# peterWon/D-LIOM

Measured on AMD Instinct MI355X. Metric: scans/sec (64-beam x 1024 pts -> 10 cm 3D submap), higher is better.
Workload: dtype f32 transforms + u16 voxels/u64 sums (rtcsm), f64 (ceres); 1 GPU; config2 W-dense: 64x1024 scan, all returns matched (adaptive voxel filters neutralised), RTCSM3D + CeresScanMatcher3D(hi+lo) + insertion(hi+lo); N_hi=65536, N_lo=65536, C=35937, linear_window=1, angular_window=5, rescored_candidates_last=2, box_kernel_variant=0, map_scans=20, grids_inserted_into=2, parallelism=replicas x1

## Files before the change

### d-liom_amd/csrc/rtcsm3d.hip

```cpp
#include <algorithm>
#include <cmath>
#include <cstdlib>
#include <cstring>
#include <type_traits>
#include <vector>

#include <dlfcn.h>
#include <rccl/rccl.h>

#include "device_common.h"
#include "host_math.h"
#include "probability_values.h"
#include "score_box.h"

namespace dliom {

constexpr int kBlock = 256;

template <int PPT, bool WIDE = false>
__global__ __launch_bounds__(kBlock) void rtcsm_score_kernel(
    GridView g, const float* __restrict__ px, const float* __restrict__ py,
    const float* __restrict__ pz, const float4* __restrict__ rot, int R, int r_first, int r_last,
    const float* __restrict__ trans, int T, int rots_per_block,
    unsigned long long* __restrict__ sums) {
  extern __shared__ unsigned block_sum[];
  float x[PPT], y[PPT], z[PPT];
#pragma unroll
  for (int k = 0; k < PPT; ++k) {
    const int i = (blockIdx.x * PPT + k) * kBlock + threadIdx.x;
    x[k] = px[i];
    y[k] = py[i];
    z[k] = pz[i];
  }
  const int r_begin = r_first + blockIdx.y * rots_per_block;
  const int r_end = min(r_begin + rots_per_block, r_last);
  const int lane = threadIdx.x & 63;
  const float inv = g.inv_resolution;
  typedef typename std::conditional<WIDE, unsigned long long, unsigned>::type idx_t;
  const idx_t sentinel = static_cast<idx_t>(1) << (3 * g.log2_leaves);
  const unsigned lb = static_cast<unsigned>(g.log2_leaves);
  for (int r = r_begin; r < r_end; ++r) {
    for (int j = threadIdx.x; j < T; j += kBlock) block_sum[j] = 0u;
    __syncthreads();
    const float4 qq = rot[r];
// ... 578 lines not shown
    }
  }
  std::vector<unsigned> bitmap(static_cast<size_t>(passes) * kBitmapWords, 0u);
  const unsigned thr_units = static_cast<unsigned>(s_units + B);
  for (int tp = 0; tp < passes; ++tp) {
    const Pass& ps = pass[static_cast<size_t>(tp)];
    for (int a = 0; a < 3; ++a) {
      unsigned* words = bitmap.data() + static_cast<size_t>(tp) * kBitmapWords + static_cast<size_t>(a) * (kBuckets / 32);
      for (int jj = 0; jj < ps.tc; ++jj) {
        const double tv = static_cast<double>(tau[(static_cast<size_t>(tp) * TC + jj) * 4 + a]);
        const double af = tv - std::floor(tv);
        const double L = -af - 1.5 * u, H = -af + (thr_units + 1.5) * u;
        const long long b0 = static_cast<long long>(std::floor(L * kBuckets)), b1 = static_cast<long long>(std::floor(H * kBuckets));
        for (long long b = b0; b <= b1; ++b) {
          const unsigned m = static_cast<unsigned>(((b % kBuckets) + kBuckets) % kBuckets);
          words[m >> 5] |= 1u << (m & 31u);
        }
      }
    }
  }
  {
    const double step = c.w.angular_step_size;
    const double a_lanes = (2.0 * c.w.angular_window_size + 1.0) * step;
    const double spread = a_lanes * 0.6 * cloud.max_norm / res;
    const double dim = spread + 2.0 * taumax + 8.0;
    if (dim > kMaxDim || dim * dim * (dim * 0.25) > cells) return (ctx->last_box_refusal = DLIOM_BOX_REFUSED_WINDOW, DLIOM_ERR_CAPACITY);
  }
  const int rot_groups_all = (r_last - r_first + 63) / 64;
  static const int forced_nw = env_int("DLIOM_BOX_NW", 0);
  const int nw = forced_nw >= 1 && forced_nw <= kWaves
                     ? std::min(forced_nw, rot_groups_all)
                     : std::min(rot_groups_all, kWaves);
  const int rot_blocks = (rot_groups_all + nw - 1) / nw;
  if (TC * sizeof(float4) + kBitmapWords * 4 + 16 + static_cast<size_t>(nw) * kListWords * 4 + static_cast<size_t>(cells) * 2 >
      160 * 1024)
    return (ctx->last_box_refusal = DLIOM_BOX_REFUSED_LDS, DLIOM_ERR_CAPACITY);
  struct GroupCache {
    int A = -1, r_first = -1, r_last = -1, nw = 0;
    float step = 0.f;
    std::vector<Group> groups;
  };
  static thread_local GroupCache gcache;
  const bool gcache_hit = gcache.A == c.w.angular_window_size && gcache.step == c.w.angular_step_size &&
                          gcache.r_first == r_first && gcache.r_last == r_last && gcache.nw == nw;
  std::vector<Group>& groups = gcache.groups;
  if (!gcache_hit) {
    gcache.A = -1;
    groups.assign(static_cast<size_t>(rot_blocks), Group());
  }
  for (size_t gi = 0; !gcache_hit && gi < groups.size(); ++gi) {
    Group& gr = groups[gi];
    const int r0 = r_first + static_cast<int>(gi) * nw * 64;
    const int cnt = std::max(0, std::min(nw * 64, r_last - r0));
    gr.c_lane = cnt / 2;
    gr.theta2 = 0.f;
    for (int a = 0; a < 3; ++a) gr.dc[a] = gr.hd[a] = 0.f;
    if (cnt <= 0) {
      gr.c_lane = 0;
      continue;
    }
    auto qd = [&](int r, double q[4]) {
      const QF& f = c.rot_raw[static_cast<size_t>(r)];
      const double nn = std::sqrt(double(f.w) * f.w + double(f.x) * f.x + double(f.y) * f.y + double(f.z) * f.z);
      q[0] = f.w / nn; q[1] = f.x / nn; q[2] = f.y / nn; q[3] = f.z / nn;
    };
    double qc[4];
    qd(r0 + gr.c_lane, qc);
// ... 2 lines not shown
      double q[4];
      qd(r0 + l, q);
      const double a0 = qc[0], a1 = -qc[1], a2 = -qc[2], a3 = -qc[3];
      double dq[4] = {a0 * q[0] - a1 * q[1] - a2 * q[2] - a3 * q[3], a0 * q[1] + a1 * q[0] + a2 * q[3] - a3 * q[2],
                      a0 * q[2] - a1 * q[3] + a2 * q[0] + a3 * q[1], a0 * q[3] + a1 * q[2] - a2 * q[1] + a3 * q[0]};
      if (dq[0] < 0) for (double& v : dq) v = -v;
      const double vn = std::sqrt(dq[1] * dq[1] + dq[2] * dq[2] + dq[3] * dq[3]);
      const double ang = 2.0 * std::atan2(vn, dq[0]);
      const double k = vn > 1e-300 ? ang / vn : 2.0;
      const double dv[3] = {k * dq[1], k * dq[2], k * dq[3]};
      th = std::max(th, ang);
      for (int a = 0; a < 3; ++a) {
        lo3[a] = std::min(lo3[a], dv[a]);
        hi3[a] = std::max(hi3[a], dv[a]);
      }
    }
    if (th > 0.3) return (ctx->last_box_refusal = DLIOM_BOX_REFUSED_WINDOW, DLIOM_ERR_CAPACITY);
    for (int a = 0; a < 3; ++a) {
      gr.dc[a] = static_cast<float>(0.5 * (lo3[a] + hi3[a]));
      gr.hd[a] = static_cast<float>(0.5 * (hi3[a] - lo3[a]) * 1.0001 + 1e-7);
    }
    gr.theta2 = static_cast<float>(0.51 * th * th * 1.01 + 1e-9);
  }
  gcache.A = c.w.angular_window_size;
  gcache.step = c.w.angular_step_size;
  gcache.r_first = r_first;
  gcache.r_last = r_last;
  gcache.nw = nw;
  struct SpanGuard {
    dliom_ctx* c;
    int span;
    ~SpanGuard() { c->end_span(span); }
  } span_guard{ctx, ctx->begin_span(DLIOM_KERNEL_RTCSM_SCORE)};
  const size_t tau_bytes = align256(tau.size() * 4);
  const size_t pass_only_bytes = align256(pass.size() * sizeof(Pass));
  const size_t group_bytes = align256(groups.size() * sizeof(Group));
  const size_t bitmap_bytes = align256(bitmap.size() * 4);
  const size_t pass_bytes = pass_only_bytes + group_bytes + bitmap_bytes;
  DLIOM_TRY(ctx->box_tables.reserve(tau_bytes + pass_bytes));
  char* base = static_cast<char*>(ctx->box_tables.p);
  const Group* group_src = reinterpret_cast<const Group*>(base + tau_bytes + pass_only_bytes);
  if (tau_bytes + pass_bytes <= kPinBoxTables.bytes) {
    char* h = pinned_at<char>(ctx, kPinBoxTables);
    std::memcpy(h, tau.data(), tau.size() * 4);
    std::memcpy(h + tau_bytes, pass.data(), pass.size() * sizeof(Pass));
    std::memcpy(h + tau_bytes + pass_only_bytes, groups.data(), groups.size() * sizeof(Group));
    std::memcpy(h + tau_bytes + pass_only_bytes + group_bytes, bitmap.data(), bitmap.size() * 4);
    if (prep_add(prep, base, h, tau_bytes + pass_bytes, 0u))
      group_src = reinterpret_cast<const Group*>(h + tau_bytes + pass_only_bytes);
    else
      DLIOM_HIP_TRY(hipMemcpyAsync(base, h, tau_bytes + pass_bytes, hipMemcpyHostToDevice, ctx->stream));
  } else {
    DLIOM_HIP_TRY(hipMemcpyAsync(base, tau.data(), tau.size() * 4, hipMemcpyHostToDevice, ctx->stream));
    DLIOM_HIP_TRY(hipMemcpyAsync(base + tau_bytes, pass.data(), pass.size() * sizeof(Pass), hipMemcpyHostToDevice, ctx->stream));
    DLIOM_HIP_TRY(hipMemcpyAsync(base + tau_bytes + pass_only_bytes, groups.data(), groups.size() * sizeof(Group),
                                 hipMemcpyHostToDevice, ctx->stream));
    DLIOM_HIP_TRY(hipMemcpyAsync(base + tau_bytes + pass_only_bytes + group_bytes, bitmap.data(), bitmap.size() * 4,
                                 hipMemcpyHostToDevice, ctx->stream));
    DLIOM_HIP_TRY(hipStreamSynchronize(ctx->stream));
  }
  Params p;
  p.tau = reinterpret_cast<const float4*>(base);
  p.pass = reinterpret_cast<const Pass*>(base + tau_bytes);
  p.group = reinterpret_cast<const Group*>(base + tau_bytes + pass_only_bytes);
  p.bitmap = reinterpret_cast<const unsigned*>(base + tau_bytes + pass_only_bytes + group_bytes);
  p.trans = d.trans;
  p.rot = d.rot;
  p.sums = d_sums;
  p.error = d_error;
  p.R = R;
  p.r_first = r_first;
  p.r_last = r_last;
  p.T = T;
  p.passes = passes;
  p.n = n;
  p.chunk = std::min(kMaxChunk, std::max(4, chunk_pts & ~3));
  p.order = p.chunk == kCostChunk ? cloud.d_chunk_order : (p.chunk == kCostChunkBig ? cloud.d_chunk_order_big : nullptr);
  p.point_chunks = (n + p.chunk - 1) / p.chunk;
  const int rot_groups = (r_last - r_first + 63) / 64;
  p.rot_groups = rot_groups;
  p.rot_blocks = rot_blocks;
  p.nw = nw;
  p.thr = thr_units;
  p.cells = cells;
  static const int split_points = env_int("DLIOM_BOX_SPLIT", 1);
  p.split_points = split_points;
#ifdef DLIOM_EXPERIMENTS
  static const int box_debug = env_int("DLIOM_BOX_DEBUG", 0);
  p.debug = box_debug;
  if (box_debug & 512) p.order = nullptr;
#else
  p.debug = 0;
#endif
  const size_t lds = TC * sizeof(float4) + kBitmapWords * 4 + 16 + static_cast<size_t>(nw) * kListWords * 4 +
                     static_cast<size_t>(cells) * 2;
  if (lds > 160 * 1024) return (ctx->last_box_refusal = DLIOM_BOX_REFUSED_LDS, DLIOM_ERR_CAPACITY);
  typedef void (*BoxKernel)(GridView, Params, const float*, const float*, const float*);
  const BoxKernel kernel = variant == 0 ? rtcsm_score_box_kernel : (variant == 1 ? rtcsm_score_box_kernel_w3 : rtcsm_score_box_kernel_wide);
  const unsigned attr_bit = variant == 0 ? kFuncAttrScoreBox : (variant == 1 ? kFuncAttrScoreBoxW3 : kFuncAttrScoreBoxWide);
  if ((ctx->func_attr_set & attr_bit) == 0u) {
    DLIOM_HIP_TRY(hipFuncSetAttribute(reinterpret_cast<const void*>(kernel), hipFuncAttributeMaxDynamicSharedMemorySize, 160 * 1024));
    ctx->func_attr_set |= attr_bit;
  }
  ctx->last_box_variant = variant;
  static thread_local size_t resident_lds = 0;
  static thread_local int resident = 0, resident_nw = 0, resident_variant = -1;
  if (resident_lds != lds || resident_nw != nw || resident_variant != variant) {
    resident_nw = nw;
    resident_variant = variant;
    DLIOM_HIP_TRY(hipOccupancyMaxActiveBlocksPerMultiprocessor(&resident, reinterpret_cast<const void*>(kernel), 64 * nw, lds));
    resident_lds = lds;
  }
  const int want_blocks = std::max(1, resident) * ctx->num_cus;
  int slot_quads = std::max(1, want_blocks / std::max(1, rot_blocks * passes));
  slot_quads = std::min(slot_quads, p.point_chunks);
  p.slots = slot_quads;
  p.units = passes * rot_blocks;
  DLIOM_TRY(ctx->box_counters.reserve(static_cast<size_t>(passes) * rot_blocks * 4 + 256));
  if (!prep_add(prep, ctx->box_counters.p, nullptr, static_cast<size_t>(passes) * rot_blocks * 4, 0u))
    DLIOM_HIP_TRY(hipMemsetAsync(ctx->box_counters.p, 0, static_cast<size_t>(passes) * rot_blocks * 4, ctx->stream));
  p.counters = ctx->box_counters.as<unsigned>();
  p.ext_stride = static_cast<int>(cloud.n_padded);
  DLIOM_TRY(ctx->box_extents.reserve(static_cast<size_t>(rot_blocks) * 6 * static_cast<size_t>(cloud.n_padded) * 4));
  p.ext = ctx->box_extents.as<float>();
  {
    PrepArgs none;
    none.n = 0;
    const PrepArgs& jobs = prep != nullptr ? *prep : none;
    const unsigned prep_rows = jobs.n > 0 ? 1u : 0u;
    hipLaunchKernelGGL(rtcsm_box_extent_kernel, dim3(static_cast<unsigned>((n + 255) / 256), static_cast<unsigned>(rot_blocks) + prep_rows),
                       dim3(256), 0, ctx->stream, p, g.inv_resolution, cloud.d_xs, cloud.d_ys, cloud.d_zs, ctx->box_extents.as<float>(),
                       group_src, d.rot_src, jobs);
    if (prep != nullptr) prep->n = 0;
  }
  const unsigned blocks = static_cast<unsigned>(slot_quads) * passes * rot_blocks;
  hipLaunchKernelGGL(kernel, dim3(blocks), dim3(64 * nw), lds, ctx->stream, g, p, cloud.d_xs, cloud.d_ys, cloud.d_zs);
  DLIOM_HIP_TRY(hipGetLastError());
#ifdef DLIOM_TEST_HOOKS
  if (ctx->tuning[DLIOM_TUNE_RESERVED_TEST_HOOK] == 1) {
    ctx->tuning[DLIOM_TUNE_RESERVED_TEST_HOOK] = 0;
    DLIOM_HIP_TRY(hipMemsetAsync(static_cast<char*>(ctx->box_error.p) + 4, 1, 1, ctx->stream));
  }
#endif
  return DLIOM_OK;
}

constexpr int kScoreTargetBlocks = 8192;

static int launch_score_dense(dliom_ctx* ctx, const dliom_cloud& cloud, const GridView& g, const Candidates& c,
                              const DeviceCandidates& d, int r_first, int r_last, unsigned long long* d_sums,
                              int64_t* processed) {
  const int R = static_cast<int>(c.w.num_rotations), T = static_cast<int>(c.w.num_translations);
  const int n = static_cast<int>(cloud.n);
  const int Rs = r_last - r_first;
  const size_t trans_lds = static_cast<size_t>(T) * 16;
  if (trans_lds > 100 * 1024) return DLIOM_ERR_INVALID_ARGUMENT;
  int bs = kDenseMaxBlock;
  for (int cand = kDenseMaxBlock; cand >= 64; cand -= 64)
    if ((Rs + cand - 1) / cand * cand < (Rs + bs - 1) / bs * bs) bs = cand;
  if (static_cast<int64_t>((Rs + bs - 1) / bs) * ((n + 63) / 64) < 256) bs = 64;
  const int rot_groups = (Rs + bs - 1) / bs;
  int chunk = 4096;
  while (chunk > 8 && static_cast<int64_t>(rot_groups) * ((n + chunk - 1) / chunk) < kScoreTargetBlocks) chunk >>= 1;
  const int point_chunks = (n + chunk - 1) / chunk;
  *processed = static_cast<int64_t>(point_chunks) * chunk;
  DenseDomain dom;
  dom.lo = 0;
  dom.size = g.dense_stride;
// ... 753 lines not shown
```

### d-liom_amd/csrc/score_box.h

```cpp
#ifndef DLIOM_CSRC_SCORE_BOX_H_
#define DLIOM_CSRC_SCORE_BOX_H_

#include "device_common.h"

namespace dliom {
namespace box {

constexpr int kTC = 27;
#if !defined(DLIOM_EXPERIMENTS) || !defined(DLIOM_BOX_TC_WIDE)
#undef DLIOM_BOX_TC_WIDE
#define DLIOM_BOX_TC_WIDE 49
#endif
constexpr int kTCWide = DLIOM_BOX_TC_WIDE;
#if !defined(DLIOM_EXPERIMENTS) || !defined(DLIOM_BOX_MAX_WAVES)
#undef DLIOM_BOX_MAX_WAVES
#define DLIOM_BOX_MAX_WAVES 4
#endif
constexpr int kWaves = DLIOM_BOX_MAX_WAVES;
constexpr int kMaxDim = 120;
constexpr int kMaxChunk = 64;
constexpr int kBuckets = 8192;
constexpr int kBitmapWords = 3 * kBuckets / 32;
constexpr int kL1Cap = 320;
constexpr int kL2Cap = 128;
#ifndef DLIOM_BOX_HOT_P
#define DLIOM_BOX_HOT_P 4
#endif
constexpr int kHotP = DLIOM_BOX_HOT_P;
#if !defined(DLIOM_EXPERIMENTS) || !defined(DLIOM_BOX_EXP)
#undef DLIOM_BOX_EXP
#define DLIOM_BOX_EXP 0
#endif
#ifdef DLIOM_EXPERIMENTS
#define DLIOM_BOX_DBG(p, bit) (((p).debug & (bit)) != 0)
#define DLIOM_BOX_STAT(p, cond, k, v)                                                                \
  do {                                                                                                \
    if (((p).debug & 128) && (cond)) atomicAdd((p).error + 8 + (k), static_cast<unsigned>(v));        \
  } while (0)
#else
#define DLIOM_BOX_DBG(p, bit) false
#define DLIOM_BOX_STAT(p, cond, k, v) do { } while (0)
#endif
#ifndef DLIOM_BOX_PIPE
#define DLIOM_BOX_PIPE 1
#endif
#ifndef DLIOM_BOX_LATE_ACC
#define DLIOM_BOX_LATE_ACC 1
#endif
constexpr int kPipe = DLIOM_BOX_PIPE;
constexpr bool kLateAcc = DLIOM_BOX_LATE_ACC != 0;
constexpr int kRecords = 8;
constexpr int kListTrash = kL1Cap + kL2Cap + 4 * kRecords;
constexpr int kListWords = kListTrash + 4;

struct Pass {
  int gi[3];
  float f[3];
  float uc[3];
  float reach[3];
  int tc;
  int j0;
  int pad[2];
};

struct Group {
  int c_lane;
  float dc[3];
  float hd[3];
  float theta2;
};

struct Params {
  const float4* tau;
  const Pass* pass;
  const unsigned* bitmap;
  const float* trans;
  const float4* rot;
  const Group* group;
  const float* ext;
  int ext_stride;
  unsigned long long* sums;
  const unsigned* order;
  unsigned* counters;
  unsigned* error;
  int R, r_first, r_last, T, passes;
  int n;
  int chunk;
  int point_chunks, rot_groups, rot_blocks, nw, slots;
  int units;
  unsigned thr;
  int cells;
  int split_points;
  int debug;
};

typedef __attribute__((address_space(3))) const unsigned short lds_cu16;

__device__ __forceinline__ unsigned min_lo16(unsigned running, float w) {
  unsigned r;
  asm("v_min_u32_sdwa %0, %1, %2 dst_sel:DWORD dst_unused:UNUSED_PAD src0_sel:DWORD src1_sel:WORD_0"
      : "=v"(r)
      : "v"(running), "v"(w));
  return r;
}
__device__ __forceinline__ unsigned mad_hi16(float w, unsigned m, unsigned a) {
  unsigned r;
  asm("v_mad_u32_u16 %0, %1, %2, %3 op_sel:[1,0,0,0]" : "=v"(r) : "v"(w), "v"(m), "v"(a));
  return r;
}
typedef float float2v __attribute__((ext_vector_type(2)));
__device__ __forceinline__ float2v pk_add_lo(float2v a, float2v t) {
  float2v r;
  asm("v_pk_add_f32 %0, %1, %2 op_sel_hi:[1,0]" : "=v"(r) : "v"(a), "v"(t));
  return r;
}
__device__ __forceinline__ float2v pk_add_hi(float2v a, float2v t) {
  float2v r;
  asm("v_pk_add_f32 %0, %1, %2 op_sel:[0,1] op_sel_hi:[1,1]" : "=v"(r) : "v"(a), "v"(t));
  return r;
}
__device__ __forceinline__ unsigned to_vgpr(unsigned s) {
  unsigned v;
  asm volatile("v_mov_b32 %0, %1" : "=v"(v) : "s"(s));
  return v;
}
__device__ __forceinline__ float to_vgpr_f(float s) {
  float v;
// ... 41 lines not shown
                                           const float* __restrict__ px, const float* __restrict__ py,
                                           const float* __restrict__ pz, const Lists& ls, int base1, int n2, int rot0,
                                           int lane) {
  DLIOM_BOX_STAT(p, lane == 0, 6, n2);
  for (int e0 = 0; e0 < n2; e0 += 64) {
    const int e = e0 + lane;
    if (e < n2) {
      const unsigned item = ls.l2[e];
      const unsigned ent = ls.l1[base1 + static_cast<int>(item & 0xFFu)];
      const int j = static_cast<int>(item >> 8);
      const int* rc = ls.rec + 4 * static_cast<int>((ent >> 12) & (kRecords - 1));
      const int r = rot0 + static_cast<int>(ent & 63u), pt = rc[3] + static_cast<int>((ent >> 6) & 63u);
      const float4 qq = p.rot[r];
      const Quat4 q{qq.x, qq.y, qq.z, qq.w};
      float rx, ry, rz;
      rotate_point(q, px[pt], py[pt], pz[pt], rx, ry, rz);
      const float4 t = lds_tau[j];
      const float ax = __builtin_fmaf(rx, g.inv_resolution, static_cast<float>(ps.gi[0] - rc[0]) + ps.f[0]) + t.x;
      const float ay = __builtin_fmaf(ry, g.inv_resolution, static_cast<float>(ps.gi[1] - rc[1]) + ps.f[1]) + t.y;
      const float az = __builtin_fmaf(rz, g.inv_resolution, static_cast<float>(ps.gi[2] - rc[2]) + ps.f[2]) + t.z;
      const int fx = static_cast<int>((__float_as_uint(ax) >> 16) - 0x4300u) + rc[0];
      const int fy = static_cast<int>((__float_as_uint(ay) >> 16) - 0x4300u) + rc[1];
      const int fz = static_cast<int>((__float_as_uint(az) >> 16) - 0x4300u) + rc[2];
      const float* tr = p.trans + 3 * (ps.j0 + j);
      const int ex = cell_of(rx + tr[0], g.resolution), ey = cell_of(ry + tr[1], g.resolution),
                ez = cell_of(rz + tr[2], g.resolution);
      if (ex != fx || ey != fy || ez != fz) {
        if (abs(ex - fx) > 1 || abs(ey - fy) > 1 || abs(ez - fz) > 1) {
          atomicOr(p.error, 1u);
          atomicOr(p.error + 1, 1u);
        }
        const long long delta = static_cast<long long>(mirror_value(g, ex, ey, ez)) -
                                static_cast<long long>(mirror_value(g, fx, fy, fz));
        if (delta != 0)
          atomicAdd(&p.sums[static_cast<size_t>(ps.j0 + j) * p.R + r], static_cast<unsigned long long>(delta));
      }
    }
  }
}

__device__ __forceinline__ void resolve_l1(const GridView& g, const Params& p, const Pass& ps, const float4* lds_tau,
                                           const float* __restrict__ px, const float* __restrict__ py,
                                           const float* __restrict__ pz, const Lists& ls, int base1, int count, int rot0,
                                           int lane) {
  const bool have = lane < count;
  DLIOM_BOX_STAT(p, lane == 0, 4, 1);
  DLIOM_BOX_STAT(p, lane == 0, 5, count);
  float wx = 200.5f, wy = 200.5f, wz = 200.5f;
  if (have) {
    const unsigned ent = ls.l1[base1 + lane];
    const int* rc = ls.rec + 4 * static_cast<int>((ent >> 12) & (kRecords - 1));
    const int r = rot0 + static_cast<int>(ent & 63u), pt = rc[3] + static_cast<int>((ent >> 6) & 63u);
    const float4 qq = p.rot[r];
    const Quat4 q{qq.x, qq.y, qq.z, qq.w};
    float rx, ry, rz;
    rotate_point(q, px[pt], py[pt], pz[pt], rx, ry, rz);
    wx = __builtin_fmaf(rx, g.inv_resolution, static_cast<float>(ps.gi[0] - rc[0]) + ps.f[0]);
    wy = __builtin_fmaf(ry, g.inv_resolution, static_cast<float>(ps.gi[1] - rc[1]) + ps.f[1]);
    wz = __builtin_fmaf(rz, g.inv_resolution, static_cast<float>(ps.gi[2] - rc[2]) + ps.f[2]);
  }
  int n2 = 0;
  for (int j = 0; j < ps.tc; ++j) {
    const float4 t = lds_tau[j];
    unsigned m = min_lo16(0xFFFFFFFFu, wx + t.x);
    m = min_lo16(m, wy + t.y);
    m = min_lo16(m, wz + t.z);
    const bool mine = have && m <= p.thr;
    const unsigned long long mask = __builtin_amdgcn_ballot_w64(mine);
// ... 178 lines not shown
        acc[j - kPipe] += s;
        asm volatile("" : "+v"(acc[j - kPipe]));
      }
      if (kLateAcc) __builtin_amdgcn_sched_barrier(0);
      unsigned v[P];
#if DLIOM_BOX_EXP == 1
#pragma unroll
      for (int k = 0; k < P; ++k) v[k] = a[k] & 0x7fffu;
#else
#pragma unroll
      for (int k = 0; k < P; ++k) v[k] = *reinterpret_cast<lds_cu16*>(a[k]);
#endif
#pragma unroll
      for (int d = kPipe - 1; d > 0; --d)
#pragma unroll
        for (int k = 0; k < P; ++k) pv[d][k] = pv[d - 1][k];
#pragma unroll
      for (int k = 0; k < P; ++k) pv[0][k] = v[k];
      t = tn;
      __builtin_amdgcn_sched_barrier(0);
    }
#pragma unroll
    for (int d = kPipe - 1; d >= 0; --d) {
      unsigned s = pv[d][0];
#pragma unroll
      for (int k = 1; k < P; ++k) s += pv[d][k];
      acc[TC - 1 - d] += s;
      asm volatile("" : "+v"(acc[TC - 1 - d]));
    }
  }
  return i;
}

constexpr int kFlushPoints = 131072;
template <int TC>
__device__ __forceinline__ void flush_acc(const Params& p, const Pass& ps, unsigned (&acc)[TC], int r, bool lane_active) {
#pragma unroll
  for (int j = 0; j < TC; ++j) {
    if (lane_active && j < ps.tc && acc[j] != 0u)
      atomicAdd(&p.sums[static_cast<size_t>(ps.j0 + j) * p.R + r], static_cast<unsigned long long>(acc[j]));
    acc[j] = 0u;
  }
}

__device__ __forceinline__ bool box_geometry(const GridView& g, const Params& p, const Pass& ps, const float (&l3)[3],
                                             const float (&h3)[3], int n, int lane, Geometry& geo) {
  const bool have = lane < n;
  bool fits = true;
#pragma unroll
  for (int a = 0; a < 3; ++a) {
    const float l = fmaxf(wave_min_f(have ? l3[a] : 3.0e38f) - ps.reach[a], -1.0e6f);
    const float h = fminf(wave_max_f(have ? h3[a] : -3.0e38f) + ps.reach[a], 1.0e6f);
    geo.lo[a] = __builtin_amdgcn_readfirstlane(static_cast<int>(floorf(l)));
    geo.dim[a] = __builtin_amdgcn_readfirstlane(static_cast<int>(floorf(h))) - geo.lo[a] + 1;
  }
  {
    const int m_lo = (geo.lo[0] + g.dense_off[0]) & ~3;
    const int m_hi = geo.lo[0] + g.dense_off[0] + geo.dim[0];
    geo.lo[0] = m_lo - g.dense_off[0];
    geo.dim[0] = ((m_hi - m_lo) + 3) & ~3;
  }
  geo.sx = static_cast<unsigned>(geo.dim[0]);
  if (((geo.sx >> 2) & 1u) == 0u) geo.sx += 4u;
  const unsigned sy = static_cast<unsigned>(geo.dim[1]) | 1u;
  geo.sxy = geo.sx * sy;
#pragma unroll
  for (int a = 0; a < 3; ++a) {
    fits = fits && geo.dim[a] <= kMaxDim && abs(ps.gi[a] - geo.lo[a]) < 1000;
    geo.kb[a] = static_cast<float>(ps.gi[a] - geo.lo[a]) + ps.f[a];
  }
  fits = fits && static_cast<long long>(geo.sxy) * geo.dim[2] <= p.cells && geo.sxy <= 32767u;
  return fits;
}
// ... 29 lines not shown
    rabs[4] = fabsf(1.f - 2.f * (x * x + z * z));
    rabs[5] = fabsf(2.f * (y * z - w * x));
    rabs[6] = fabsf(2.f * (x * z - w * y));
    rabs[7] = fabsf(2.f * (y * z + w * x));
    rabs[8] = fabsf(1.f - 2.f * (x * x + y * y));
  }
  const float x = px[i], y = py[i], z = pz[i];
  const float sx_ = grp.dc[1] * z - grp.dc[2] * y, sy_ = grp.dc[2] * x - grp.dc[0] * z, sz_ = grp.dc[0] * y - grp.dc[1] * x;
  float cx, cy, cz;
  rotate_point(qc, x + sx_, y + sy_, z + sz_, cx, cy, cz);
  const float fx = fabsf(x), fy = fabsf(y), fz = fabsf(z);
  const float hx = grp.hd[1] * fz + grp.hd[2] * fy, hy = grp.hd[2] * fx + grp.hd[0] * fz, hz = grp.hd[0] * fy + grp.hd[1] * fx;
  const float m2 = grp.theta2 * (fx + fy + fz) + 1.0e-5f * (fx + fy + fz);
  const float c3[3] = {cx, cy, cz};
  float* out = ext + static_cast<size_t>(rb) * 6 * p.ext_stride + i;
#pragma unroll
  for (int a = 0; a < 3; ++a) {
    const float he = rabs[3 * a] * hx + rabs[3 * a + 1] * hy + rabs[3 * a + 2] * hz + m2;
    out[static_cast<size_t>(2 * a) * p.ext_stride] = (c3[a] - he) * inv;
    out[static_cast<size_t>(2 * a + 1) * p.ext_stride] = (c3[a] + he) * inv;
  }
}

template <int TC>
__device__ __forceinline__ void score_box_body(const GridView& g, const Params& p, const float* __restrict__ px,
                                               const float* __restrict__ py, const float* __restrict__ pz) {
  extern __shared__ float4 lds_dyn4[];
  float4* lds_tau = lds_dyn4;
  unsigned* lds_bitmap = reinterpret_cast<unsigned*>(lds_dyn4 + TC);
  const int wave = __builtin_amdgcn_readfirstlane(static_cast<int>(threadIdx.x >> 6)), lane = threadIdx.x & 63, nthreads = blockDim.x;
  typedef __attribute__((address_space(3))) char lds_char;
  const unsigned lds0 = static_cast<unsigned>(reinterpret_cast<size_t>((lds_char*)lds_dyn4));
  const unsigned tick_off = static_cast<unsigned>(TC * sizeof(float4)) + kBitmapWords * 4u;
  const unsigned lists_off = tick_off + 16u;
  const unsigned box_off = lists_off + static_cast<unsigned>(p.nw) * kListWords * 4u;
  const unsigned box_base = lds0 + box_off;
  unsigned short* box = reinterpret_cast<unsigned short*>(reinterpret_cast<char*>(lds_dyn4) + box_off);
  unsigned* tick = reinterpret_cast<unsigned*>(reinterpret_cast<char*>(lds_dyn4) + tick_off);
  Lists ls;
  ls.l1 = reinterpret_cast<unsigned*>(reinterpret_cast<char*>(lds_dyn4) + lists_off) + wave * kListWords;
  ls.l2 = ls.l1 + kL1Cap;
  ls.rec = reinterpret_cast<int*>(ls.l2 + kL2Cap);
  ls.n1 = 0;
  ls.seq = 0;
  unsigned acc[TC];
#pragma unroll
  for (int j = 0; j < TC; ++j) acc[j] = 0u;
  const int S = g.dense_stride, B = g.dense_bricks;
#ifdef DLIOM_EXPERIMENTS
  unsigned long long stamp_begin = 0ull;
  unsigned stamp_tickets = 0u;
  if (DLIOM_BOX_DBG(p, 256)) stamp_begin = wall_clock64();
#endif
  const int home = static_cast<int>(blockIdx.x % static_cast<unsigned>(p.units));
  const int slot = static_cast<int>(blockIdx.x / static_cast<unsigned>(p.units));
  int parity = 0;
  int loaded_pass = -1;
  const int hops = DLIOM_BOX_DBG(p, 64) ? 1 : p.units;
  for (int hop = 0; hop < hops; ++hop) {
    int unit = home + hop;
    if (unit >= p.units) unit -= p.units;
    unsigned* counter = p.counters + unit;
    int ticket, chunk_id;
    if (hop == 0) {
      ticket = DLIOM_BOX_DBG(p, 8) ? p.point_chunks : slot;
      chunk_id = (p.order != nullptr && ticket < p.point_chunks) ? static_cast<int>(p.order[ticket]) : ticket;
    } else {
      if (threadIdx.x == 0) {
        const int t = p.slots + static_cast<int>(atomicAdd(counter, 1u));
        tick[parity] = static_cast<unsigned>(t);
        tick[2 + parity] = (p.order != nullptr && t < p.point_chunks) ? p.order[t] : static_cast<unsigned>(t);
      }
      __syncthreads();
      ticket = static_cast<int>(tick[parity]);
      chunk_id = static_cast<int>(tick[2 + parity]);
      parity ^= 1;
    }
    if (ticket >= p.point_chunks) continue;
    const int rb = unit % p.rot_blocks;
    const int tp = unit / p.rot_blocks;
    if (tp != loaded_pass) {
      __syncthreads();
      if (threadIdx.x < TC) lds_tau[threadIdx.x] = p.tau[tp * TC + threadIdx.x];
      for (int w = threadIdx.x; w < kBitmapWords; w += nthreads) lds_bitmap[w] = p.bitmap[tp * kBitmapWords + w];
      __syncthreads();
      loaded_pass = tp;
    }
    const int rot_b0 = p.r_first + rb * p.nw * 64;
    const int groups_here = (p.r_last - rot_b0 + 63) >> 6;
    const int split = (p.split_points != 0 && p.nw == 4) ? (groups_here == 1 ? 4 : (groups_here == 2 ? 2 : 1)) : 1;
    const int rot_group = split == 4 ? 0 : (split == 2 ? (wave & 1) : wave);
    const int slice = split == 4 ? wave : (split == 2 ? (wave >> 1) : 0);
    const int rot0 = rot_b0 + rot_group * 64;
    const bool wave_active = rot0 < p.r_last && slice < split;
    const Pass ps = p.pass[tp];
    const bool lane_active = rot0 + lane < p.r_last;
    const float4 qq = p.rot[lane_active ? rot0 + lane : (wave_active ? rot0 : rot_b0)];
    const Quat4 q{qq.x, qq.y, qq.z, qq.w};
    const float* ext_rb = p.ext + static_cast<size_t>(rb) * 6 * p.ext_stride;
    int n_guess = p.chunk;
    int since_flush = 0;
    while (ticket < p.point_chunks) {
      unsigned next_raw = 0u, next_chunk = 0u;
      bool drawn = false;
#ifdef DLIOM_EXPERIMENTS
      ++stamp_tickets;
#endif
      {
        const int c = __builtin_amdgcn_readfirstlane(chunk_id);
        const int c_begin = c * p.chunk, c_end = min(c_begin + p.chunk, p.n);
        int lo = c_begin;
// ... 41 lines not shown
          DLIOM_BOX_STAT(p, threadIdx.x == 0, 0, 1);
          DLIOM_BOX_STAT(p, threadIdx.x == 0, 1, (geo.dim[0] >> 2) * geo.dim[1] * geo.dim[2]);
          DLIOM_BOX_STAT(p, threadIdx.x == 0, 2, n);
          __syncthreads();
          if (!DLIOM_BOX_DBG(p, 2)) {
            const unsigned quads = static_cast<unsigned>(geo.dim[0]) >> 2, dim1 = static_cast<unsigned>(geo.dim[1]);
            const unsigned total = __umul24(__umul24(quads, dim1), static_cast<unsigned>(geo.dim[2]));
            const float inv_q = 1.0f / static_cast<float>(quads), inv_dy = 1.0f / static_cast<float>(dim1);
            const int bx0 = geo.lo[0] + g.dense_off[0], by0 = geo.lo[1] + g.dense_off[1], bz0 = geo.lo[2] + g.dense_off[2];
            const unsigned uB = static_cast<unsigned>(B), uBB = __umul24(uB, uB), uS = static_cast<unsigned>(S);
            const char* dense_bytes = reinterpret_cast<const char*>(g.dense);
#pragma unroll 4
            for (unsigned e = threadIdx.x; e < total; e += static_cast<unsigned>(nthreads)) {
              const unsigned row = static_cast<unsigned>((static_cast<float>(e) + 0.5f) * inv_q);
              const unsigned xq = e - __umul24(row, quads);
              const unsigned z = static_cast<unsigned>((static_cast<float>(row) + 0.5f) * inv_dy);
              const unsigned y = row - __umul24(z, dim1);
              const int mx = bx0 + static_cast<int>(4u * xq), my = by0 + static_cast<int>(y), mz = bz0 + static_cast<int>(z);
              unsigned long long val = 0x0001000100010001ull;
              if (static_cast<unsigned>(mx) < 4u * uB && static_cast<unsigned>(my) < uS && static_cast<unsigned>(mz) < uS) {
                const unsigned umx = static_cast<unsigned>(mx), umy = static_cast<unsigned>(my), umz = static_cast<unsigned>(mz);
                const unsigned off = ((__umul24(umz >> 2, uBB) + __umul24(umy >> 2, uB) + (umx >> 2)) << 7) |
                                     (((umz & 3u) << 5) | ((umy & 3u) << 3));
                val = *reinterpret_cast<const unsigned long long*>(dense_bytes + off);
              }
              *reinterpret_cast<unsigned long long*>(box + (__umul24(z, geo.sxy) + __umul24(y, geo.sx) + 4u * xq)) = val;
            }
          }
          const unsigned rec_id = static_cast<unsigned>(ls.seq & (kRecords - 1));
          if (lane < 4) ls.rec[4 * rec_id + lane] = lane < 3 ? geo.lo[lane] : lo;
          ++ls.seq;
          __syncthreads();
          if (drawn && threadIdx.x == 0) {
            const int t = p.slots + static_cast<int>(next_raw);
            next_chunk = (p.order != nullptr && t < p.point_chunks) ? p.order[t] : static_cast<unsigned>(t);
          }
          if (wave_active && !DLIOM_BOX_DBG(p, 4)) {
            const int part = split > 1 ? ((((n + split - 1) >> (split == 4 ? 2 : 1)) + 3) & ~3) : n;
            const int s_lo = lo + min(n, slice * part), s_n = min(n, (slice + 1) * part) - min(n, slice * part);
            int i = s_lo;
            const int e8 = kHotP == 8 ? s_lo + (s_n & ~7) : s_lo, e4 = s_lo + (s_n & ~3), e1 = s_lo + s_n;
            for (;;) {
              if (kHotP == 8 && i < e8)
                i = main_loop<kHotP, TC>(g, p, geo, q, px, py, pz, i, e8, lo, lds_tau, lds_bitmap, box_base, ls, rec_id, lane_active, lane, acc);
              if (i >= e8 && i < e4)
                i = main_loop<4, TC>(g, p, geo, q, px, py, pz, i, e4, lo, lds_tau, lds_bitmap, box_base, ls, rec_id, lane_active, lane, acc);
              if (i >= e4 && i < e1)
                i = main_loop<1, TC>(g, p, geo, q, px, py, pz, i, e1, lo, lds_tau, lds_bitmap, box_base, ls, rec_id, lane_active, lane, acc);
              if (i >= e1) break;
              drain_l1(g, p, ps, lds_tau, px, py, pz, ls, false, rot0, lane);
            }
            if (!DLIOM_BOX_DBG(p, 1) && (ls.n1 >= 64 || (ls.seq & (kRecords - 1)) == 0))
              drain_l1(g, p, ps, lds_tau, px, py, pz, ls, (ls.seq & (kRecords - 1)) == 0, rot0, lane);
          }
          lo += n;
        }
      }
      if (threadIdx.x == 0) {
        if (!drawn) {
          const int t = p.slots + static_cast<int>(atomicAdd(counter, 1u));
          next_raw = static_cast<unsigned>(t - p.slots);
          next_chunk = (p.order != nullptr && t < p.point_chunks) ? p.order[t] : static_cast<unsigned>(t);
        }
        tick[parity] = static_cast<unsigned>(p.slots) + next_raw;
        tick[2 + parity] = next_chunk;
      }
      __syncthreads();
      ticket = static_cast<int>(tick[parity]);
      chunk_id = static_cast<int>(tick[2 + parity]);
      parity ^= 1;
    }
    if (wave_active && !DLIOM_BOX_DBG(p, 1)) drain_l1(g, p, ps, lds_tau, px, py, pz, ls, true, rot0, lane);
    ls.n1 = 0;
    if (DLIOM_BOX_DBG(p, 16)) {
#pragma unroll
      for (int j = 0; j < TC; ++j) {
        if (lane_active && j < ps.tc)
          atomicAdd(&p.sums[static_cast<size_t>(ps.j0 + j) * p.R + rot0 + lane], static_cast<unsigned long long>(acc[j]));
        acc[j] = 0u;
      }
    } else if (!DLIOM_BOX_DBG(p, 32)) {
      flush_acc(p, ps, acc, rot0 + lane, lane_active);
    }
  }
#ifdef DLIOM_EXPERIMENTS
  if (DLIOM_BOX_DBG(p, 256) && threadIdx.x == 0 && blockIdx.x < 4096u) {
    unsigned long long* st = reinterpret_cast<unsigned long long*>(p.error + 64) + 4 * blockIdx.x;
    unsigned xcc;
    asm volatile("s_getreg_b32 %0, hwreg(HW_REG_XCC_ID)" : "=s"(xcc));
    st[0] = stamp_begin;
    st[1] = wall_clock64();
    st[2] = stamp_tickets;
    st[3] = xcc;
  }
#endif
}


__global__ __launch_bounds__(64 * kWaves) __attribute__((amdgpu_waves_per_eu(4, 8))) void rtcsm_score_box_kernel(
    GridView g, Params p, const float* __restrict__ px, const float* __restrict__ py, const float* __restrict__ pz) {
  score_box_body<kTC>(g, p, px, py, pz);
}
__global__ __launch_bounds__(64 * kWaves) __attribute__((amdgpu_waves_per_eu(3, 8))) void rtcsm_score_box_kernel_w3(
    GridView g, Params p, const float* __restrict__ px, const float* __restrict__ py, const float* __restrict__ pz) {
  score_box_body<kTC>(g, p, px, py, pz);
}
__global__ __launch_bounds__(64 * kWaves) __attribute__((amdgpu_waves_per_eu(3, 8))) void rtcsm_score_box_kernel_wide(
    GridView g, Params p, const float* __restrict__ px, const float* __restrict__ py, const float* __restrict__ pz) {
  score_box_body<kTCWide>(g, p, px, py, pz);
}

}
}

#endif
```

Measured before the change: 965.6 scans/s.

## Weight-proportional block homes and dynamic work stealing across score-box units

Replaces the uniform slot-per-unit launch layout with a host-computed table that gives each (pass, rotation-block) unit a number of resident blocks proportional to its estimated work. A small home table is uploaded with the other box tables. When a block finishes its unit, it now picks the unit with the most remaining chunks instead of hopping round-robin. The change also switches sum atomics to 32-bit when the point count guarantees no overflow. The intent is to cut load imbalance and tail idle time, at the cost of extra host-side allotment, a per-unit scan of global counters by wave 0, and more atomic contention on busy units.

```diff
diff --git a/d-liom_amd/csrc/rtcsm3d.hip b/d-liom_amd/csrc/rtcsm3d.hip
--- a/d-liom_amd/csrc/rtcsm3d.hip
+++ b/d-liom_amd/csrc/rtcsm3d.hip
@@ -10,6 +10,7 @@
 
 #include "device_common.h"
 #include "host_math.h"
+#include "score_units.h"
 #include "probability_values.h"
 #include "score_box.h"
 
@@ -654,7 +655,7 @@
                      ? std::min(forced_nw, rot_groups_all)
                      : std::min(rot_groups_all, kWaves);
   const int rot_blocks = (rot_groups_all + nw - 1) / nw;
-  if (TC * sizeof(float4) + kBitmapWords * 4 + 16 + static_cast<size_t>(nw) * kListWords * 4 + static_cast<size_t>(cells) * 2 >
+  if (TC * sizeof(float4) + kBitmapWords * 4 + kTickBytes + static_cast<size_t>(nw) * kListWords * 4 + static_cast<size_t>(cells) * 2 >
       160 * 1024)
     return (ctx->last_box_refusal = DLIOM_BOX_REFUSED_LDS, DLIOM_ERR_CAPACITY);
   struct GroupCache {
@@ -723,38 +724,7 @@
     int span;
     ~SpanGuard() { c->end_span(span); }
   } span_guard{ctx, ctx->begin_span(DLIOM_KERNEL_RTCSM_SCORE)};
-  const size_t tau_bytes = align256(tau.size() * 4);
-  const size_t pass_only_bytes = align256(pass.size() * sizeof(Pass));
-  const size_t group_bytes = align256(groups.size() * sizeof(Group));
-  const size_t bitmap_bytes = align256(bitmap.size() * 4);
-  const size_t pass_bytes = pass_only_bytes + group_bytes + bitmap_bytes;
-  DLIOM_TRY(ctx->box_tables.reserve(tau_bytes + pass_bytes));
-  char* base = static_cast<char*>(ctx->box_tables.p);
-  const Group* group_src = reinterpret_cast<const Group*>(base + tau_bytes + pass_only_bytes);
-  if (tau_bytes + pass_bytes <= kPinBoxTables.bytes) {
-    char* h = pinned_at<char>(ctx, kPinBoxTables);
-    std::memcpy(h, tau.data(), tau.size() * 4);
-    std::memcpy(h + tau_bytes, pass.data(), pass.size() * sizeof(Pass));
-    std::memcpy(h + tau_bytes + pass_only_bytes, groups.data(), groups.size() * sizeof(Group));
-    std::memcpy(h + tau_bytes + pass_only_bytes + group_bytes, bitmap.data(), bitmap.size() * 4);
-    if (prep_add(prep, base, h, tau_bytes + pass_bytes, 0u))
-      group_src = reinterpret_cast<const Group*>(h + tau_bytes + pass_only_bytes);
-    else
-      DLIOM_HIP_TRY(hipMemcpyAsync(base, h, tau_bytes + pass_bytes, hipMemcpyHostToDevice, ctx->stream));
-  } else {
-    DLIOM_HIP_TRY(hipMemcpyAsync(base, tau.data(), tau.size() * 4, hipMemcpyHostToDevice, ctx->stream));
-    DLIOM_HIP_TRY(hipMemcpyAsync(base + tau_bytes, pass.data(), pass.size() * sizeof(Pass), hipMemcpyHostToDevice, ctx->stream));
-    DLIOM_HIP_TRY(hipMemcpyAsync(base + tau_bytes + pass_only_bytes, groups.data(), groups.size() * sizeof(Group),
-                                 hipMemcpyHostToDevice, ctx->stream));
-    DLIOM_HIP_TRY(hipMemcpyAsync(base + tau_bytes + pass_only_bytes + group_bytes, bitmap.data(), bitmap.size() * 4,
-                                 hipMemcpyHostToDevice, ctx->stream));
-    DLIOM_HIP_TRY(hipStreamSynchronize(ctx->stream));
-  }
   Params p;
-  p.tau = reinterpret_cast<const float4*>(base);
-  p.pass = reinterpret_cast<const Pass*>(base + tau_bytes);
-  p.group = reinterpret_cast<const Group*>(base + tau_bytes + pass_only_bytes);
-  p.bitmap = reinterpret_cast<const unsigned*>(base + tau_bytes + pass_only_bytes + group_bytes);
   p.trans = d.trans;
   p.rot = d.rot;
   p.sums = d_sums;
@@ -783,7 +753,7 @@
 #else
   p.debug = 0;
 #endif
-  const size_t lds = TC * sizeof(float4) + kBitmapWords * 4 + 16 + static_cast<size_t>(nw) * kListWords * 4 +
+  const size_t lds = TC * sizeof(float4) + kBitmapWords * 4 + kTickBytes + static_cast<size_t>(nw) * kListWords * 4 +
                      static_cast<size_t>(cells) * 2;
   if (lds > 160 * 1024) return (ctx->last_box_refusal = DLIOM_BOX_REFUSED_LDS, DLIOM_ERR_CAPACITY);
   typedef void (*BoxKernel)(GridView, Params, const float*, const float*, const float*);
@@ -805,8 +775,59 @@
   const int want_blocks = std::max(1, resident) * ctx->num_cus;
   int slot_quads = std::max(1, want_blocks / std::max(1, rot_blocks * passes));
   slot_quads = std::min(slot_quads, p.point_chunks);
-  p.slots = slot_quads;
+  p.add32 = n <= kFlushPoints ? 1 : 0;
   p.units = passes * rot_blocks;
+  std::vector<double> unit_weights(static_cast<size_t>(p.units));
+  for (int u = 0; u < p.units; ++u) {
+    const int rot_b0 = r_first + (u % rot_blocks) * nw * 64;
+    unit_weights[static_cast<size_t>(u)] = unit_weight((r_last - rot_b0 + 63) >> 6, nw, p.split_points);
+  }
+  std::vector<int> slots_per_unit;
+  std::vector<UnitHome> homes;
+  const unsigned blocks = static_cast<unsigned>(allot_homes(unit_weights, slot_quads * p.units, p.point_chunks, &slots_per_unit, &homes));
+  std::vector<unsigned> unit_slots(static_cast<size_t>(unit_slots_words(p.units)), 0u);
+  for (int u = 0; u < p.units; ++u) unit_slots[static_cast<size_t>(u)] = static_cast<unsigned>(slots_per_unit[static_cast<size_t>(u)]);
+  const size_t tau_bytes = align256(tau.size() * 4);
+  const size_t pass_only_bytes = align256(pass.size() * sizeof(Pass));
+  const size_t group_bytes = align256(groups.size() * sizeof(Group));
+  const size_t bitmap_bytes = align256(bitmap.size() * 4);
+  static_assert((kBitmapWords * 4) % 256 == 0 && sizeof(UnitHome) == 8, "unit_slots() finds the table behind the bitmaps");
+  const size_t unit_slot_bytes = static_cast<size_t>(unit_slots_words(p.units)) * 4;
+  const size_t unit_bytes = align256(unit_slot_bytes + homes.size() * sizeof(UnitHome));
+  const size_t pass_bytes = pass_only_bytes + group_bytes + bitmap_bytes + unit_bytes;
+  DLIOM_TRY(ctx->box_tables.reserve(tau_bytes + pass_bytes));
+  char* base = static_cast<char*>(ctx->box_tables.p);
+  const Group* group_src = reinterpret_cast<const Group*>(base + tau_bytes + pass_only_bytes);
+  if (tau_bytes + pass_bytes <= kPinBoxTables.bytes) {
+    char* h = pinned_at<char>(ctx, kPinBoxTables);
+    std::memcpy(h, tau.data(), tau.size() * 4);
+    std::memcpy(h + tau_bytes, pass.data(), pass.size() * sizeof(Pass));
+    std::memcpy(h + tau_bytes + pass_only_bytes, groups.data(), groups.size() * sizeof(Group));
+    std::memcpy(h + tau_bytes + pass_only_bytes + group_bytes, bitmap.data(), bitmap.size() * 4);
+    std::memcpy(h + tau_bytes + pass_only_bytes + group_bytes + bitmap_bytes, unit_slots.data(), unit_slots.size() * 4);
+    std::memcpy(h + tau_bytes + pass_only_bytes + group_bytes + bitmap_bytes + unit_slot_bytes, homes.data(),
+                homes.size() * sizeof(UnitHome));
+    if (prep_add(prep, base, h, tau_bytes + pass_bytes, 0u))
+      group_src = reinterpret_cast<const Group*>(h + tau_bytes + pass_only_bytes);
+    else
+      DLIOM_HIP_TRY(hipMemcpyAsync(base, h, tau_bytes + pass_bytes, hipMemcpyHostToDevice, ctx->stream));
+  } else {
+    DLIOM_HIP_TRY(hipMemcpyAsync(base, tau.data(), tau.size() * 4, hipMemcpyHostToDevice, ctx->stream));
+    DLIOM_HIP_TRY(hipMemcpyAsync(base + tau_bytes, pass.data(), pass.size() * sizeof(Pass), hipMemcpyHostToDevice, ctx->stream));
+    DLIOM_HIP_TRY(hipMemcpyAsync(base + tau_bytes + pass_only_bytes, groups.data(), groups.size() * sizeof(Group),
+                                 hipMemcpyHostToDevice, ctx->stream));
+    DLIOM_HIP_TRY(hipMemcpyAsync(base + tau_bytes + pass_only_bytes + group_bytes, bitmap.data(), bitmap.size() * 4,
+                                 hipMemcpyHostToDevice, ctx->stream));
+    DLIOM_HIP_TRY(hipMemcpyAsync(base + tau_bytes + pass_only_bytes + group_bytes + bitmap_bytes, unit_slots.data(),
+                                 unit_slots.size() * 4, hipMemcpyHostToDevice, ctx->stream));
+    DLIOM_HIP_TRY(hipMemcpyAsync(base + tau_bytes + pass_only_bytes + group_bytes + bitmap_bytes + unit_slot_bytes, homes.data(),
+                                 homes.size() * sizeof(UnitHome), hipMemcpyHostToDevice, ctx->stream));
+    DLIOM_HIP_TRY(hipStreamSynchronize(ctx->stream));
+  }
+  p.tau = reinterpret_cast<const float4*>(base);
+  p.pass = reinterpret_cast<const Pass*>(base + tau_bytes);
+  p.group = reinterpret_cast<const Group*>(base + tau_bytes + pass_only_bytes);
+  p.bitmap = reinterpret_cast<const unsigned*>(base + tau_bytes + pass_only_bytes + group_bytes);
   DLIOM_TRY(ctx->box_counters.reserve(static_cast<size_t>(passes) * rot_blocks * 4 + 256));
   if (!prep_add(prep, ctx->box_counters.p, nullptr, static_cast<size_t>(passes) * rot_blocks * 4, 0u))
     DLIOM_HIP_TRY(hipMemsetAsync(ctx->box_counters.p, 0, static_cast<size_t>(passes) * rot_blocks * 4, ctx->stream));
@@ -824,7 +845,6 @@
                        group_src, d.rot_src, jobs);
     if (prep != nullptr) prep->n = 0;
   }
-  const unsigned blocks = static_cast<unsigned>(slot_quads) * passes * rot_blocks;
   hipLaunchKernelGGL(kernel, dim3(blocks), dim3(64 * nw), lds, ctx->stream, g, p, cloud.d_xs, cloud.d_ys, cloud.d_zs);
   DLIOM_HIP_TRY(hipGetLastError());
 #ifdef DLIOM_TEST_HOOKS
diff --git a/d-liom_amd/csrc/score_box.h b/d-liom_amd/csrc/score_box.h
--- a/d-liom_amd/csrc/score_box.h
+++ b/d-liom_amd/csrc/score_box.h
@@ -52,6 +52,7 @@
 constexpr int kRecords = 8;
 constexpr int kListTrash = kL1Cap + kL2Cap + 4 * kRecords;
 constexpr int kListWords = kListTrash + 4;
+constexpr int kTickBytes = 32;
 
 struct Pass {
   int gi[3];
@@ -86,13 +87,24 @@
   int R, r_first, r_last, T, passes;
   int n;
   int chunk;
-  int point_chunks, rot_groups, rot_blocks, nw, slots;
+  int point_chunks, rot_groups, rot_blocks, nw;
+  int add32;
   int units;
   unsigned thr;
   int cells;
   int split_points;
   int debug;
 };
+
+__host__ __device__ __forceinline__ int unit_slots_words(int units) { return (units + 3) & ~3; }
+__device__ __forceinline__ const unsigned* unit_slots(const Params& p) { return p.bitmap + p.passes * kBitmapWords; }
+__device__ __forceinline__ const uint2* unit_homes(const Params& p) {
+  return reinterpret_cast<const uint2*>(unit_slots(p) + unit_slots_words(p.units));
+}
+
+constexpr int kFlushPoints = 131072;
+static_assert(static_cast<unsigned long long>(kFlushPoints) * 0x7fffull <= 0xffffffffull,
+              "kFlushPoints values of at most 0x7fff (the mask of a grid value) fit an accumulator and a 32-bit sum");
 
 typedef __attribute__((address_space(3))) const unsigned short lds_cu16;
 
@@ -200,8 +212,13 @@
         }
         const long long delta = static_cast<long long>(mirror_value(g, ex, ey, ez)) -
                                 static_cast<long long>(mirror_value(g, fx, fy, fz));
-        if (delta != 0)
-          atomicAdd(&p.sums[static_cast<size_t>(ps.j0 + j) * p.R + r], static_cast<unsigned long long>(delta));
+        if (delta != 0) {
+          unsigned long long* sum = &p.sums[static_cast<size_t>(ps.j0 + j) * p.R + r];
+          if (p.add32 != 0)
+            atomicAdd(reinterpret_cast<unsigned*>(sum), static_cast<unsigned>(delta));
+          else
+            atomicAdd(sum, static_cast<unsigned long long>(delta));
+        }
       }
     }
   }
@@ -446,13 +463,18 @@
   return i;
 }
 
-constexpr int kFlushPoints = 131072;
 template <int TC>
 __device__ __forceinline__ void flush_acc(const Params& p, const Pass& ps, unsigned (&acc)[TC], int r, bool lane_active) {
+  const bool add32 = p.add32 != 0;
 #pragma unroll
   for (int j = 0; j < TC; ++j) {
-    if (lane_active && j < ps.tc && acc[j] != 0u)
-      atomicAdd(&p.sums[static_cast<size_t>(ps.j0 + j) * p.R + r], static_cast<unsigned long long>(acc[j]));
+    if (lane_active && j < ps.tc && acc[j] != 0u) {
+      unsigned long long* sum = &p.sums[static_cast<size_t>(ps.j0 + j) * p.R + r];
+      if (add32)
+        atomicAdd(reinterpret_cast<unsigned*>(sum), acc[j]);
+      else
+        atomicAdd(sum, static_cast<unsigned long long>(acc[j]));
+    }
     acc[j] = 0u;
   }
 }
@@ -548,7 +570,7 @@
   typedef __attribute__((address_space(3))) char lds_char;
   const unsigned lds0 = static_cast<unsigned>(reinterpret_cast<size_t>((lds_char*)lds_dyn4));
   const unsigned tick_off = static_cast<unsigned>(TC * sizeof(float4)) + kBitmapWords * 4u;
-  const unsigned lists_off = tick_off + 16u;
+  const unsigned lists_off = tick_off + static_cast<unsigned>(kTickBytes);
   const unsigned box_off = lists_off + static_cast<unsigned>(p.nw) * kListWords * 4u;
   const unsigned box_base = lds0 + box_off;
   unsigned short* box = reinterpret_cast<unsigned short*>(reinterpret_cast<char*>(lds_dyn4) + box_off);
@@ -565,34 +587,21 @@
   const int S = g.dense_stride, B = g.dense_bricks;
 #ifdef DLIOM_EXPERIMENTS
   unsigned long long stamp_begin = 0ull;
-  unsigned stamp_tickets = 0u;
+  unsigned stamp_tickets = 0u, stamp_visits = 0u;
   if (DLIOM_BOX_DBG(p, 256)) stamp_begin = wall_clock64();
 #endif
-  const int home = static_cast<int>(blockIdx.x % static_cast<unsigned>(p.units));
-  const int slot = static_cast<int>(blockIdx.x / static_cast<unsigned>(p.units));
+  int unit, ticket, chunk_id;
+  {
+    const uint2 home = unit_homes(p)[blockIdx.x];
+    unit = static_cast<int>(home.x);
+    ticket = DLIOM_BOX_DBG(p, 8) ? p.point_chunks : static_cast<int>(home.y);
+    chunk_id = (p.order != nullptr && ticket < p.point_chunks) ? static_cast<int>(p.order[ticket]) : ticket;
+  }
   int parity = 0;
   int loaded_pass = -1;
-  const int hops = DLIOM_BOX_DBG(p, 64) ? 1 : p.units;
-  for (int hop = 0; hop < hops; ++hop) {
-    int unit = home + hop;
-    if (unit >= p.units) unit -= p.units;
+  for (;;) {
     unsigned* counter = p.counters + unit;
-    int ticket, chunk_id;
-    if (hop == 0) {
-      ticket = DLIOM_BOX_DBG(p, 8) ? p.point_chunks : slot;
-      chunk_id = (p.order != nullptr && ticket < p.point_chunks) ? static_cast<int>(p.order[ticket]) : ticket;
-    } else {
-      if (threadIdx.x == 0) {
-        const int t = p.slots + static_cast<int>(atomicAdd(counter, 1u));
-        tick[parity] = static_cast<unsigned>(t);
-        tick[2 + parity] = (p.order != nullptr && t < p.point_chunks) ? p.order[t] : static_cast<unsigned>(t);
-      }
-      __syncthreads();
-      ticket = static_cast<int>(tick[parity]);
-      chunk_id = static_cast<int>(tick[2 + parity]);
-      parity ^= 1;
-    }
-    if (ticket >= p.point_chunks) continue;
+    const int slots_u = static_cast<int>(unit_slots(p)[unit]);
     const int rb = unit % p.rot_blocks;
     const int tp = unit / p.rot_blocks;
     if (tp != loaded_pass) {
@@ -700,7 +709,7 @@
           ++ls.seq;
           __syncthreads();
           if (drawn && threadIdx.x == 0) {
-            const int t = p.slots + static_cast<int>(next_raw);
+            const int t = slots_u + static_cast<int>(next_raw);
             next_chunk = (p.order != nullptr && t < p.point_chunks) ? p.order[t] : static_cast<unsigned>(t);
           }
           if (wave_active && !DLIOM_BOX_DBG(p, 4)) {
@@ -726,18 +735,21 @@
       }
       if (threadIdx.x == 0) {
         if (!drawn) {
-          const int t = p.slots + static_cast<int>(atomicAdd(counter, 1u));
-          next_raw = static_cast<unsigned>(t - p.slots);
+          const int t = slots_u + static_cast<int>(atomicAdd(counter, 1u));
+          next_raw = static_cast<unsigned>(t - slots_u);
           next_chunk = (p.order != nullptr && t < p.point_chunks) ? p.order[t] : static_cast<unsigned>(t);
         }
-        tick[parity] = static_cast<unsigned>(p.slots) + next_raw;
+        tick[parity] = static_cast<unsigned>(slots_u) + next_raw;
         tick[2 + parity] = next_chunk;
       }
       __syncthreads();
-      ticket = static_cast<int>(tick[parity]);
+      ticket = __builtin_amdgcn_readfirstlane(static_cast<int>(tick[parity]));
       chunk_id = static_cast<int>(tick[2 + parity]);
       parity ^= 1;
     }
+#ifdef DLIOM_EXPERIMENTS
+    ++stamp_visits;
+#endif
     if (wave_active && !DLIOM_BOX_DBG(p, 1)) drain_l1(g, p, ps, lds_tau, px, py, pz, ls, true, rot0, lane);
     ls.n1 = 0;
     if (DLIOM_BOX_DBG(p, 16)) {
@@ -750,6 +762,38 @@
     } else if (!DLIOM_BOX_DBG(p, 32)) {
       flush_acc(p, ps, acc, rot0 + lane, lane_active);
     }
+    if (DLIOM_BOX_DBG(p, 8 | 64)) break;
+    do {
+      if (wave == 0) {
+        const unsigned* slots = unit_slots(p);
+        int most = 0, where = -1;
+        for (int u = lane; u < p.units; u += 64) {
+          const int left = p.point_chunks - static_cast<int>(slots[u]) -
+                           static_cast<int>(__hip_atomic_load(p.counters + u, __ATOMIC_RELAXED, __HIP_MEMORY_SCOPE_AGENT));
+          if (left > most) most = left, where = u;
+        }
+        const float top = wave_max_f(static_cast<float>(most));
+        const unsigned long long who = __builtin_amdgcn_ballot_w64(most > 0 && static_cast<float>(most) == top);
+        const int first = who != 0ull ? __builtin_ctzll(who) : 0;
+        const int u = __shfl(where, first);
+        if (lane == 0) {
+          unsigned t = 0u, c = 0u;
+          if (who != 0ull) {
+            t = slots[u] + atomicAdd(p.counters + u, 1u);
+            c = (p.order != nullptr && t < static_cast<unsigned>(p.point_chunks)) ? p.order[t] : t;
+          }
+          tick[parity] = t;
+          tick[2 + parity] = c;
+          tick[4 + parity] = who != 0ull ? static_cast<unsigned>(u) : 0xFFFFFFFFu;
+        }
+      }
+      __syncthreads();
+      ticket = __builtin_amdgcn_readfirstlane(static_cast<int>(tick[parity]));
+      chunk_id = static_cast<int>(tick[2 + parity]);
+      unit = __builtin_amdgcn_readfirstlane(static_cast<int>(tick[4 + parity]));
+      parity ^= 1;
+    } while (unit >= 0 && ticket >= p.point_chunks);
+    if (unit < 0) break;
   }
 #ifdef DLIOM_EXPERIMENTS
   if (DLIOM_BOX_DBG(p, 256) && threadIdx.x == 0 && blockIdx.x < 4096u) {
@@ -759,7 +803,7 @@
     st[0] = stamp_begin;
     st[1] = wall_clock64();
     st[2] = stamp_tickets;
-    st[3] = xcc;
+    st[3] = (xcc & 0xFu) | (static_cast<unsigned long long>(stamp_visits) << 8);
   }
 #endif
 }
diff --git a/d-liom_amd/csrc/score_units.h b/d-liom_amd/csrc/score_units.h
--- /dev/null
+++ b/d-liom_amd/csrc/score_units.h
@@ -0,0 +1,63 @@
+#ifndef DLIOM_CSRC_SCORE_UNITS_H_
+#define DLIOM_CSRC_SCORE_UNITS_H_
+
+#include <algorithm>
+#include <vector>
+
+namespace dliom {
+namespace box {
+
+struct UnitHome {
+  unsigned unit;
+  unsigned slot;
+};
+
+inline int unit_split(int groups_here, int nw, int split_points) {
+  return (split_points != 0 && nw == 4) ? (groups_here == 1 ? 4 : (groups_here == 2 ? 2 : 1)) : 1;
+}
+inline double unit_weight(int groups_here, int nw, int split_points) {
+  if (groups_here >= nw) return 1.0;
+  if (split_points != 0) return 1.0 / unit_split(groups_here, nw, split_points);
+  return static_cast<double>(std::max(1, groups_here)) / nw;
+}
+
+inline int allot_homes(const std::vector<double>& weight, int launch, int cap, std::vector<int>* slots,
+                       std::vector<UnitHome>* homes) {
+  const int units = static_cast<int>(weight.size());
+  slots->assign(static_cast<size_t>(units), 0);
+  homes->clear();
+  if (units == 0) return 0;
+  cap = std::max(cap, 1);
+  const long long room = static_cast<long long>(units) * cap;
+  const int target = static_cast<int>(std::min<long long>(std::max(launch, units), room));
+  double sum = 0.0;
+  for (double w : weight) sum += w;
+  std::vector<double> quota(static_cast<size_t>(units));
+  int total = 0;
+  for (int u = 0; u < units; ++u) {
+    quota[u] = (static_cast<double>(target) * weight[u]) / sum;
+    (*slots)[u] = static_cast<int>(std::min<double>(std::max(quota[u], 1.0), static_cast<double>(cap)));
+    total += (*slots)[u];
+  }
+  while (total != target) {
+    int best = -1;
+    for (int u = 0; u < units; ++u) {
+      if (total < target ? (*slots)[u] >= cap : (*slots)[u] <= 1) continue;
+      const double d = quota[u] - (*slots)[u], db = best < 0 ? 0.0 : quota[best] - (*slots)[best];
+      if (best < 0 || (total < target ? d > db : d < db)) best = u;
+    }
+    (*slots)[best] += total < target ? 1 : -1;
+    total += total < target ? 1 : -1;
+  }
+  homes->reserve(static_cast<size_t>(target));
+  const int rounds = *std::max_element(slots->begin(), slots->end());
+  for (int s = 0; s < rounds; ++s)
+    for (int u = 0; u < units; ++u)
+      if (s < (*slots)[u]) homes->push_back(UnitHome{static_cast<unsigned>(u), static_cast<unsigned>(s)});
+  return target;
+}
+
+}
+}
+
+#endif
```

After: 975.3 scans/s, median of 6. About the same (+1.0%).
